# SchlomoFeng/GDN

Hardware: AMD Instinct MI355X
Metric: sliding-windows/sec forward+anomaly-score, SWaT-shape (127 sensors, W=15) (higher is better)
Workload: dtype f32; 1 GPU; BASELINE configs[2]: SWaT-shape eval forward + anomaly score; sensors=127, window=15, topk=30, dim=64, out_layer_num=1, batch=512, batches_per_launch=64, windows_per_launch=32768, storage=fp32, multi_gpu_measured=False, hip_graph=True, forward_streams=3, parallelism=single GPU

## Files before the change

gdn_amd/_lib.py:

```python
from __future__ import annotations

import ctypes
import functools
import os

_HERE = os.path.dirname(os.path.abspath(__file__))
LIB_PATH = os.environ.get("GDN_HIP_LIB", os.path.join(_HERE, "libgdn_hip.so"))
ABI_VERSION = 23

_c_int, _c_float, _p = ctypes.c_int, ctypes.c_float, ctypes.c_void_p

SIGNATURES = {
    "gdn_abi_version": [],
    "gdn_nbr_pitch": [_c_int],
    "gdn_topk_graph": [_p, _c_int, _c_int, _c_int, _p, _p, _p, _p, _p],
    "gdn_graph_from_topk": [_p, _c_int, _c_int, _p, _p, _p],
    "gdn_node_terms": [_p, _p, _p, _p, _p, _p, _c_int, _c_int, _c_int, _p, _p],
    "gdn_bn_fold": [_p, _p, _p, _p, _c_float, _c_int, _p, _p],
    "gdn_project_fwd": [_p, _p, _p, _c_int, _c_int, _c_int, _c_int, _p, _p, _p, _p],
    "gdn_project_fwd_series": [_p, _c_int, _c_int, _p, _p, _c_int, _c_int, _c_int, _c_int, _p, _p, _p, _p],
    "gdn_tile_fits": [_c_int] * 4,
    "gdn_kernel_family": [_c_int] * 6,
    "gdn_tile_forward_form": [_c_int] * 5,
    "gdn_terms_pitch": [_c_int],
    "gdn_attn_aggregate_fwd": [_p, _p, _p, _p, _p, _p, _c_int, _c_int, _c_int, _c_int, _p, _p, _p],
    "gdn_head_fwd": [_p, _p, _p, _p, _p, _p, _c_int, _c_int, _c_int, _p, _p, _p],
    "gdn_head_train_fwd": [_p] * 10 + [_c_float] + [_c_int] * 3 + [_c_float] * 4 + [_p] * 9,
    "gdn_head_train_workspace_bytes": [_c_int, _c_int],
    "gdn_head_train_stats_bytes": [_c_int],
    "gdn_exact_sum_workspace_bytes": [],
    "gdn_exact_sum": [_p, _c_int, _p, _p, _p],
    "gdn_head_train_bwd": [_p] * 10 + [_c_float, _p] + [_c_int] * 3 + [_c_float] * 2 + [_p] * 10,
    "gdn_head_train_fwd_rng": [_p] * 9 + [_c_float] + [_c_int] * 3 + [_c_float] * 4 + [_p] * 8 + [_c_int, _p],
    "gdn_head_train_bwd_rng": [_p] * 9 + [_c_float, _p] + [_c_int] * 3 + [_c_float] * 2 + [_p] * 9 + [_c_int, _p],
    "gdn_head_train_fwd_act": [_p] * 8 + [_c_float, _p, _c_float] + [_c_int] * 3 + [_c_float] * 4 + [_p] * 8 + [_c_int, _p],
    "gdn_head_train_bwd_act": [_p] * 9 + [_c_float, _p, _c_float, _p] + [_c_int] * 3 + [_c_float] * 2 + [_p] * 7 + [_c_int, _p],
    "gdn_mlp_train_saved_bytes": [_c_int] * 4,
    "gdn_mlp_train_workspace_bytes": [_c_int] * 4,
    "gdn_mlp_train_fwd": [_p] * 8 + [_c_int] * 4 + [_p] * 4,
    "gdn_mlp_train_bwd": [_p] * 4 + [_c_int] * 4 + [_p] * 7,
    "gdn_mlp_eval_workspace_bytes": [_c_int] * 4,
    "gdn_mlp_eval_fwd": [_p] * 6 + [_c_int] * 4 + [_p] * 3,
    "gdn_topk_graph_terms": [_p, _c_int, _c_int, _c_int] + [_p] * 8 + [_c_int, _p, _p],
    "gdn_forward_fused_plan_keys": [_p] * 4 + [_c_int] * 7 + [_p, _p],
    "gdn_forward_fused_series_plan_keys": [_p, _c_int, _c_int] + [_p] * 3 + [_c_int] * 6 + [_p, _p],
    "gdn_attn_aggregate_bwd_uses_reverse": [_c_int] * 3,
    "gdn_head_mse_workspace_bytes": [],
    "gdn_head_train_fwd_rng_mse": [_p] * 9 + [_c_float] + [_c_int] * 3 + [_c_float] * 4 + [_p] * 12 + [_c_int, _p],
    "gdn_project_bwd_partials": [_p] * 4 + [_c_int] * 4 + [_p, _p, _p],
    "gdn_train_finish": [_p, _p] + [_c_int] * 4 + [_p] * 8 + [_c_int, _c_int] + [_p] * 4,
    "gdn_adam_step": [_p] * 5 + [_c_int] + [ctypes.c_double] * 6 + [_c_int, _c_int, _p],
    "gdn_terms_bwd_acc": [_p] * 8 + [_c_int] * 3 + [_p] * 6 + [_c_int, _p],
    "gdn_mse_workspace_bytes": [],
    "gdn_mse_loss_grad": [_p, _p, ctypes.c_longlong, _p, _p, _p, _p],
    "gdn_forward_fused": [_p] * 11 + [_c_int] * 5 + [_p, _p],
    "gdn_forward_fused_series": [_p, _c_int, _c_int] + [_p] * 10 + [_c_int] * 5 + [_p, _p],
    "gdn_mlp_plan_bytes": [_c_int] * 3,
    "gdn_mlp_plan_layer": [_p] * 6 + [_c_float] + [_c_int] * 4 + [_p, _p],
    "gdn_mlp_plan_out": [_p, _p] + [_c_int] * 3 + [_p, _p],
    "gdn_mlp_fwd": [_p, _p] + [_c_int] * 4 + [_p, _p],
    "gdn_head_mlp_fwd": [_p] * 5 + [_c_int] * 5 + [_p, _p],
    "gdn_fused_plan_bytes": [_c_int] * 5,
    "gdn_fused_plan_build": [_p] * 10 + [_c_int] * 5 + [_p, _p],
    "gdn_forward_fused_plan": [_p, _p] + [_c_int] * 6 + [_p, _p, _p],
    "gdn_forward_fused_series_plan": [_p, _c_int, _c_int, _p] + [_c_int] * 5 + [_p, _p, _p],
    "gdn_fused_plan_limit_offset": [_c_int] * 5,
    "gdn_graph_bank_order": [_p, _c_int, _c_int, _p, _p],
    "gdn_forward_fused_gated": [_p] * 12 + [_c_int] * 5 + [_p, _p],
    "gdn_forward_fused_series_gated": [_p, _p, _c_int, _c_int] + [_p] * 10 + [_c_int] * 5 + [_p, _p],
    "gdn_project_fwd_wide": [_p, _p, _p, _c_int, _c_int, _c_int, _c_int, _p, _p, _p, _p],
    "gdn_attn_aggregate_fwd_wide": [_p, _p, _p, _p, _p, _p, _c_int, _c_int, _c_int, _c_int, _p, _p, _p],
    "gdn_attn_aggregate_bwd_wide": [_p] * 8 + [_c_int] * 4 + [_p] * 6,
    "gdn_project_fwd_bf16": [_p, _p, _p, _c_int, _c_int, _c_int, _c_int, _p, _p, _p, _p],
    "gdn_attn_aggregate_fwd_bf16": [_p, _p, _p, _p, _p, _p, _c_int, _c_int, _c_int, _c_int, _p, _p, _p],
    "gdn_head_fwd_bf16": [_p, _p, _p, _p, _p, _p, _c_int, _c_int, _c_int, _p, _p, _p],
    "gdn_forward_fused_bf16": [_p] * 11 + [_c_int] * 5 + [_p, _p],
    "gdn_attn_aggregate_bwd": [_p] * 8 + [_c_int] * 4 + [_p] * 6,
    "gdn_attn_aggregate_bwd_workspace_bytes": [_c_int] * 4,
    "gdn_train_supported": [_c_int] * 4,
    "gdn_rev_pitch": [_c_int],
    "gdn_graph_reverse": [_p, _p, _c_int, _c_int, _p, _p, _p],
    "gdn_project_bwd_workspace_bytes": [_c_int, _c_int, _c_int],
    "gdn_project_bwd": [_p] * 4 + [_c_int] * 4 + [_p] * 5,
    "gdn_terms_bwd": [_p] * 8 + [_c_int] * 3 + [_p] * 7,
    "gdn_score_workspace_bytes": [_c_int, _c_int],
    "gdn_score_select_workspace_bytes": [_c_int, _c_int, _c_int],
    "gdn_score_keys": [_p, _p, _c_int, _c_int, _c_int, _p, _p],
    "gdn_score_select": [_p, _c_int, _c_int, _c_int, ctypes.c_longlong, _p, _p, _p],
    "gdn_score_select_paths": [_p, _c_int, _c_int, _c_int, ctypes.c_longlong, _p, _p, _p, _p],
    "gdn_score_quantiles": [_p, _p, _c_int, _c_int, _p, _p, _p],
    "gdn_score_smooth_max": [_p, _p, _p, _c_int, _c_int, _c_int, _p, _p, _p, _p, _p],
    "gdn_score_smooth_topm": [_p, _p, _p, _c_int, _c_int, _c_int, _p, _p, _c_int, _p, _p, _p],
    "gdn_series_fill_workspace_bytes": [_c_int, _c_int],
    "gdn_series_fill": [_p] + [_c_int] * 3 + [_p] * 7,
    "gdn_score_keys_keep": [_p, _p, _p, _c_int, _c_int, _c_int, _p, _p],
    "gdn_score_smooth_max_gaps": [_p, _p, _p, _c_int, _c_int, _c_int, _p, _p, _p, _p, _p, _p, _p],
    "gdn_score_smooth_topm_gaps": [_p, _p, _p, _c_int, _c_int, _c_int, _p, _p, _c_int, _p, _p, _p, _p, _p],
    "gdn_attention_workspace_bytes": [_c_int] * 4,
    "gdn_attention_mean": [_p, ctypes.c_longlong, ctypes.c_longlong] + [_p] * 4 + [_c_int] * 4 + [_p, _p, _p],
    "gdn_attention_at": [_p, ctypes.c_longlong, _p, _p, _c_int, _p, _p, _p] + [_c_int] * 3 + [_p, _p],
    "gdn_windows_gather": [_p, _c_int, ctypes.c_longlong, _p, ctypes.c_longlong, _p, ctypes.c_longlong, _c_int, _c_int,
                           _p, _p, _p],
    "gdn_epoch_advance": [_p, _p, _p, ctypes.c_longlong, _p],
    "gdn_mse_batch_means": [_p, _p, ctypes.c_longlong, _c_int, ctypes.c_longlong, _p, _p, _p, _p],
    "gdn_windows_gather_gaps": [_p, _c_int, ctypes.c_longlong, _p, ctypes.c_longlong, _p, ctypes.c_longlong, _c_int,
                                _c_int, _p, _p, _p, _p, _p, _p],
    "gdn_mse_batch_means_masked": [_p, _p, _p, ctypes.c_longlong, _c_int, ctypes.c_longlong, _p, _p, _p, _p, _p],
    "gdn_mse_loss_grad_masked": [_p, _p, _p, _p, _c_int, _c_int, _p, _p, _p, _p, _p],
    "gdn_stream_state_bytes": [_c_int, _c_int],
    "gdn_stream_init": [_p, _p, ctypes.c_longlong, _c_int, _c_int, _p],
    "gdn_stream_windows": [_p, _p, _c_int, _c_int, _c_int, _c_int, _p, _p],
    "gdn_stream_score": [_p] * 5 + [_c_int] * 4 + [_p] * 4,
    "gdn_stream_advance": [_p] * 6 + [_c_int] * 5 + [_p, _p, ctypes.c_longlong, _p],
    "gdn_stream_fill": [_p, _p] + [_c_int] * 4 + [_p] * 4,
    "gdn_stream_score_gaps": [_p] * 6 + [_c_int] * 4 + [_p] * 4,
    "gdn_stream_advance_gaps": [_p] * 8 + [_c_int] * 5 + [_p, _p, ctypes.c_longlong, _p, _p],
    "gdn_stream_calib_bytes": [_c_int, _c_int],
    "gdn_stream_calib_write": [_p] * 4 + [_c_int] * 5 + [_p] * 3,
    "gdn_stream_calib_write_gaps": [_p] * 5 + [_c_int] * 5 + [_p] * 3,
    "gdn_score_keys_valid": [_p, _p, _p, _c_int, _c_int, _c_int, _p, _p],
    "gdn_score_key_counts": [_p, _c_int, _c_int, _c_int, _p, _p],
    "gdn_score_select_counts": [_p, _c_int, _c_int, _c_int, _p, _c_int, _p, _p, _p, _p],
    "gdn_stream_calib_write_sensor": [_p] * 5 + [_c_int] * 5 + [_p] * 3,
    "gdn_prep_stats_workspace_bytes": [ctypes.c_longlong, _c_int],
    "gdn_prep_stats": [_p, ctypes.c_longlong, _c_int, _c_int, _p, _p, _p],
    "gdn_prep_series": [_p, ctypes.c_longlong, _c_int, _c_int, _p, _p, _c_int, _p, _p, _p, _p],
    "gdn_prep_ticks": [_p, _c_int, _c_int, _p, _c_int, _p, _c_int, _c_int, _p, _p, _c_int, _p],
    "gdn_episodes_workspace_bytes": [ctypes.c_longlong, ctypes.c_longlong],
    "gdn_episodes_scan": [_p, _p, ctypes.c_longlong, _c_int, ctypes.c_double, ctypes.c_double, _c_int, _c_int,
                          ctypes.c_longlong, ctypes.c_longlong] + [_p] * 10,
    "gdn_episodes_scan_grid": [_p, _p, ctypes.c_longlong, _c_int, ctypes.c_double, ctypes.c_double, _c_int, _c_int,
                               ctypes.c_longlong, ctypes.c_longlong] + [_p] * 9 + [_c_int, _p],
    "gdn_stream_events_bytes": [_c_int, ctypes.c_longlong],
    "gdn_stream_events": [_p] * 5 + [_c_int] * 5 + [ctypes.c_longlong, _p, _p],
    "gdn_alarm_sweep": [_p, _p, ctypes.c_longlong, _p, _p, _p, _p, ctypes.c_longlong, _p, _p],
    "gdn_fleet_state_bytes": [_c_int] * 3,
    "gdn_fleet_init": [_p, _p, ctypes.c_longlong, _c_int, _c_int, _c_int, _p],
    "gdn_fleet_windows": [_p] * 3 + [_c_int] * 4 + [_p, _p],
    "gdn_fleet_score": [_p] * 6 + [_c_int] * 5 + [_p] * 4,
    "gdn_fleet_advance": [_p] * 7 + [_c_int] * 5 + [_p, _p, ctypes.c_longlong, _p],
    "gdn_fleet_fill": [_p] * 3 + [_c_int] * 4 + [_p] * 4,
    "gdn_fleet_score_gaps": [_p] * 7 + [_c_int] * 5 + [_p] * 4,
    "gdn_fleet_advance_gaps": [_p] * 9 + [_c_int] * 5 + [_p, _p, ctypes.c_longlong, _p, _p],
    "gdn_fleet_events_bytes": [_c_int, _c_int, ctypes.c_longlong],
    "gdn_fleet_events": [_p] * 6 + [_c_int] * 7 + [ctypes.c_longlong, _p, _p],
    "gdn_fleet_calib_bytes": [_c_int] * 3,
    "gdn_fleet_calib_write": [_p] * 5 + [_c_int] * 6 + [_p] * 3,
    "gdn_fleet_calib_write_gaps": [_p] * 6 + [_c_int] * 6 + [_p] * 3,
    "gdn_fleet_calib_write_sensor": [_p] * 6 + [_c_int] * 6 + [_p] * 3,
    "gdn_fleet_ring_counts": [_p, _p, _c_int, _c_int, _c_int, _p, _p, _p],
    "gdn_fleet_ring_threshold_bytes": [_c_int, _c_int],
    "gdn_fleet_ring_threshold": [_p] * 5 + [_c_int] * 5 + [ctypes.c_double, _c_int] + [_p] * 8,
    "gdn_fleet_prep_bytes": [_c_int] * 3,
    "gdn_fleet_prep_ticks": [_p, _c_int, _c_int, _p, _p] + [_c_int] * 4 + [_p] * 4,
}

FAMILY_NONE, FAMILY_DENSE, FAMILY_TILE, FAMILY_LARGE, FAMILY_LONG, FAMILY_ANY = range(6)
STAGE_PROJECT, STAGE_AGGREGATE, STAGE_ATTN_BWD, STAGE_PROJECT_BWD, STAGE_TERMS, STAGE_HEAD, STAGE_FUSED = range(7)
ROUTE_WIDE, ROUTE_BF16, ROUTE_SERIES = 1, 2, 4


@functools.lru_cache(maxsize=None)
def family(stage: int, n: int, w: int, d: int, k: int, flags: int = 0) -> int:
    return load().gdn_kernel_family(stage, n, w, d, k, flags) & 0xff


ERRORS = {-1: "GDN_ERR_ARG (null pointer or non-positive dimension)",
          -2: "GDN_ERR_LAUNCH (HIP launch failed)",
          -3: "GDN_ERR_UNSUPPORTED (shape outside the supported set, see include/gdn_hip.h)"}

_lib = None


class GdnHipError(RuntimeError):
    pass


def load() -> ctypes.CDLL:
    global _lib
    if _lib is not None:
        return _lib
    if not os.path.exists(LIB_PATH):
        raise GdnHipError(
            f"{LIB_PATH} not found: the HIP extension is not built and gdn_amd has no CPU "
            "fallback. Run `python -c \"import __graft_entry__ as g; g.build()\"` (needs hipcc).")
    lib = ctypes.CDLL(LIB_PATH)
    for name, argtypes in SIGNATURES.items():
        fn = getattr(lib, name)
        fn.argtypes = argtypes
        fn.restype = ctypes.c_longlong if name.endswith(("_bytes", "_offset")) else _c_int
    if lib.gdn_abi_version() != ABI_VERSION:
        raise GdnHipError(f"ABI mismatch: library {lib.gdn_abi_version()} != binding {ABI_VERSION}")
    _lib = lib
    return lib


def call(name: str, *args) -> None:
    rc = getattr(load(), name)(*args)
    if rc != 0:
        raise GdnHipError(f"{name} failed: {ERRORS.get(rc, rc)}")
```

gdn_amd/csrc/gdn_forward_dense.hip:

```cpp
#include "gdn_common.hpp"

#include <stdlib.h>

int gdn_dense_fused_op_d128(int op, const void* args, int bf16, unsigned* plan_out, long long* bytes,
                            hipStream_t st);

namespace {

typedef _Float16 h8 __attribute__((ext_vector_type(8)));
typedef _Float16 h2 __attribute__((ext_vector_type(2)));
typedef __bf16 b8 __attribute__((ext_vector_type(8)));
typedef __bf16 b2 __attribute__((ext_vector_type(2)));
typedef float f32x16 __attribute__((ext_vector_type(16)));
typedef unsigned int u32x4 __attribute__((ext_vector_type(4)));
typedef float f32x2 __attribute__((ext_vector_type(2)));

#ifndef GDN_TRIM_SPLIT
#define GDN_TRIM_SPLIT 1
#endif
#ifndef GDN_TRIM_RELU
#define GDN_TRIM_RELU 1
#endif
#ifndef GDN_TRIM_PACK
#define GDN_TRIM_PACK 1
#endif

template <bool PACK>
struct Pk2 {
  static __device__ __forceinline__ f32x2 mul(f32x2 a, f32x2 b) {
    if constexpr (PACK) return a * b;
    return f32x2{a[0] * b[0], a[1] * b[1]};
  }
  static __device__ __forceinline__ f32x2 mul(f32x2 a, float b) { return mul(a, f32x2{b, b}); }
  static __device__ __forceinline__ f32x2 add(f32x2 a, f32x2 b) {
    if constexpr (PACK) return a + b;
    return f32x2{a[0] + b[0], a[1] + b[1]};
  }
  static __device__ __forceinline__ f32x2 add(f32x2 a, float b) { return add(a, f32x2{b, b}); }
  static __device__ __forceinline__ f32x2 sub(f32x2 a, float b) {
    if constexpr (PACK) return a - f32x2{b, b};
    return f32x2{a[0] - b, a[1] - b};
  }
  static __device__ __forceinline__ f32x2 fma(f32x2 a, f32x2 b, f32x2 c) {
    if constexpr (PACK) return __builtin_elementwise_fma(a, b, c);
    return f32x2{__builtin_fmaf(a[0], b[0], c[0]), __builtin_fmaf(a[1], b[1], c[1])};
  }
};

__device__ __forceinline__ float relu_acc(float v) {
#if GDN_TRIM_RELU
  return __builtin_elementwise_maximum(v, 0.f);
#else
  return fmaxf(v, 0.f);
// ... 54 lines not shown
    hi = __builtin_bit_cast(unsigned, p);
    lo = __builtin_bit_cast(unsigned, l);
  }
  static __device__ __forceinline__ f32x16 mfma(u32x4 a, u32x4 b, f32x16 c) {
    return __builtin_amdgcn_mfma_f32_32x32x16_f16(__builtin_bit_cast(h8, a), __builtin_bit_cast(h8, b), c, 0, 0, 0);
  }
};

template <>
struct Fmt<FMT_BF16> {
  static __device__ __forceinline__ unsigned pk(float a, float b) {
    asm("" : "+v"(a));
    asm("" : "+v"(b));
    const b2 p = {(__bf16)a, (__bf16)b};
    return __builtin_bit_cast(unsigned, p);
  }
  static __device__ __forceinline__ float res0(unsigned p, float x) { return x - __uint_as_float(p << 16); }
  static __device__ __forceinline__ float res1(unsigned p, float x) { return x - __uint_as_float(p & 0xffff0000u); }
  static __device__ __forceinline__ void split2(float& a, float& b, unsigned& hi, unsigned& lo) {
    hi = pk(a, b);
    lo = pk(res0(hi, a), res1(hi, b));
  }
  static __device__ __forceinline__ f32x16 mfma(u32x4 a, u32x4 b, f32x16 c) {
    return __builtin_amdgcn_mfma_f32_32x32x16_bf16(__builtin_bit_cast(b8, a), __builtin_bit_cast(b8, b), c, 0, 0, 0);
  }
};

template <int FMT, int NTERM, bool TRIM = true>
__device__ __forceinline__ void split8(const float (&v)[8], u32x4 (&out)[NTERM]) {
  float r[8];
#pragma unroll
  for (int j = 0; j < 8; ++j) r[j] = v[j];
  if constexpr (NTERM == 2 && TRIM) {
#pragma unroll
    for (int j = 0; j < 4; ++j) {
      unsigned hi, lo;
      Fmt<FMT>::split2(r[2 * j], r[2 * j + 1], hi, lo);
      out[0][j] = hi;
      out[NTERM - 1][j] = lo;
    }
    return;
  }
#pragma unroll
  for (int t = 0; t < NTERM; ++t)
#pragma unroll
    for (int j = 0; j < 4; ++j) {
      const unsigned p = Fmt<FMT>::pk(r[2 * j], r[2 * j + 1]);
      out[t][j] = p;
      if (t + 1 < NTERM) {
        r[2 * j] = Fmt<FMT>::res0(p, r[2 * j]);
        r[2 * j + 1] = Fmt<FMT>::res1(p, r[2 * j + 1]);
      }
    }
}

__host__ __device__ __forceinline__ int pos_of_source(int src) {
  return (src & ~12) | ((src & 4) << 1) | ((src & 8) >> 1);
}

enum { DMODE_FUSED = 0 };

template <int NT, int DC, int WK, int SL, int FMT>
struct DCfg {
  static constexpr int KS = 2 * NT;
  static constexpr int ROWS = 32 * NT;
  static constexpr int THREADS = 64 * NT;
  static constexpr int AROW = KS * 32 + 16;
  static constexpr int AWAVE = 32 * AROW;
  static constexpr bool XAGG = FMT == FMT_F16;
  static constexpr int MCB = XAGG ? 1 : DC;
  static constexpr int NPX = FMT == FMT_F16 ? 2 : 1;
  static constexpr int NTL = FMT == FMT_F16 ? 2 : 3;
  static constexpr int NTXIN = FMT == FMT_F16 ? 2 : 1;
  static constexpr int XP = 16 * WK + 4;
  static constexpr int XU = 8 * WK;
  static constexpr bool XHALF = XAGG && WK == 1;
  static constexpr int XFL = XHALF ? 16 : 32;
  static constexpr int XFRAG = 2 * XFL * 16;
  static constexpr int OFF_A = 0;
  static constexpr int OFF_XF = NT * AWAVE;
  static constexpr int OFF_XS = OFF_XF + KS * MCB * NPX * XFRAG;
  static constexpr int OFF_SI = OFF_XS + (XAGG ? 0 : ROWS * XP * 4);
  static constexpr int OFF_SJ = OFF_SI + ROWS * 4;
  static constexpr int OFF_EC = OFF_SJ + ROWS * 4;
  static constexpr int OFF_CS = OFF_EC + 4 * 32 * DC * 4;
  static constexpr int CS_WORDS = XAGG ? 0 : 3 * ROWS;
  static constexpr bool XKFAM = XHALF && DC == 2 && SL <= 16;
  static constexpr int XKEEP_TABLE = SL <= 8 || NT == 4 ? KS : 2;
  static constexpr int XKEEP = !XKFAM ? 0 : GDN_XKEEP < 0 ? XKEEP_TABLE : GDN_XKEEP < KS ? GDN_XKEEP : KS;
  static constexpr bool BLDS = XKFAM && (GDN_BL_LDS < 0 ? SL > 8 && NT == 4 : GDN_BL_LDS != 0);
  static constexpr int OFF_BL = OFF_CS + CS_WORDS * 4;
  static constexpr int LDS = OFF_BL + (BLDS ? DC * WK * NTL * 1024 : 0);
  static constexpr int CW = 16 * WK, RS = THREADS / CW;
  static __host__ __device__ constexpr int xrow0(int xsl) { return XAGG ? 16 * (xsl >> 1) + 4 * (xsl & 1) : xsl; }
  static __host__ __device__ constexpr int xro(int u) {
    return XAGG ? 16 * NT * (u >> 3) + 8 * ((u & 7) >> 2) + (u & 3) : u * RS;
  }
  static constexpr int LDS_UNIT = 1280;
  static constexpr int LDS_ALLOC = (LDS + LDS_UNIT - 1) / LDS_UNIT * LDS_UNIT;
  static constexpr bool PACK = GDN_TRIM_PACK != 0 && SL <= 16 && FMT == FMT_F16;
  static constexpr int WGS = !(DC == 2 && NT >= 3 && SL <= 16 && WK == 1) ? 1
                             : XAGG && 3 * LDS_ALLOC <= 160 * 1024 ? 3 : 2;
};

struct DArgs {
  const void* x;
  int series_len;
  int series_first;
  int batch, n, w, pitch, d;
  const float* lin_w;
// ... 227 lines not shown
    for (int r = 0; r < 16; ++r) {
      const int c = cb * 32 + (r & 3) + 8 * (r >> 2) + 4 * h;
      k.e2[cb][r] = ld_or(a.emb, tgt * d + c, tgt < n) * a.bn2[c] *
                    (FMT == FMT_F16 ? 1.f / (GDN_F16_Z_SCALE * GDN_F16_X_SCALE) : 1.f);
    }
  k.out_b = a.out_b[0];
}

template <int NT, int DC, int FMT>
__device__ __forceinline__ void compute_tables(const DArgs& a, float* dst) {
  constexpr int ROWS = 32 * NT, THREADS = 64 * NT, d = 32 * DC;
  const int tid = threadIdx.x, n = a.n;
  for (int c = tid; c < d; c += THREADS) {
    dst[c] = a.bn2[d + c];
    dst[d + c] = a.out_w[c];
    dst[2 * d + c] = a.bn1[c];
    dst[3 * d + c] = fmaf(a.gnn_bias[c], a.bn1[c], a.bn1[d + c]) *
                     (FMT == FMT_F16 ? GDN_F16_Z_SCALE * GDN_F16_X_SCALE : 1.f);
  }
  if constexpr (FMT == FMT_F16) return;
  float* ct = dst + 4 * d;
  for (int t = tid; t < 3 * ROWS; t += THREADS) {
    const int which = t / ROWS, row = t - which * ROWS;
    float v = ld_or(a.node_terms, 2 * GDN_A_PITCH + which * n + row, which < 2 && row < n) * GDN_LOG2E;
    if (which == 1 && row == n) v = -INFINITY;
    ct[t] = v;
  }
}

template <int NT, int DC, int FMT>
__device__ __forceinline__ float compute_xlimit(const DArgs& a) {
  if constexpr (FMT != FMT_F16) return INFINITY;
  __shared__ unsigned m_lin, m_c;
  const int tid = threadIdx.x, d = 32 * DC;
  if (tid == 0) { m_lin = 0u; m_c = 0u; }
  __syncthreads();
  for (int c = tid; c < d; c += 64 * NT) {
    const float sc = a.bn1[c] * GDN_F16_X_SCALE;
    float lmax = 0.f;
    for (int q = 0; q < a.w; ++q) {
      const float v = fabsf(a.lin_w[c * a.w + q] * sc);
      lmax = v > lmax || v != v ? v : lmax;
    }
    const float cin = fabsf(fmaf(a.gnn_bias[c], a.bn1[c], a.bn1[d + c]));
    atomicMax(&m_lin, __float_as_uint(lmax));
    atomicMax(&m_c, __float_as_uint(cin));
  }
  __syncthreads();
  const float lmax = __uint_as_float(m_lin), cmax = __uint_as_float(m_c);
  if (!(lmax < 60000.f) || !(cmax < 3.0e38f)) return 0.f;
  return 60000.f / GDN_F16_XT_SCALE;
}

template <int NT, int DC, int WK, int SL, int FMT>
__global__ __launch_bounds__(64 * NT) void gdn_dense_plan_kernel(const DArgs a, unsigned* plan) {
  using K = LaneConsts<NT, DC, WK, SL, FMT>;
  constexpr int T = 64 * NT;
  __shared__ int s_sj[T][SL], s_sc[T][SL];
  __shared__ unsigned char s_perm[T][SL];
  K k;
  compute_lane_consts(a, k);
  const int tid = threadIdx.x;
#pragma unroll
  for (int q = 0; q < SL; ++q) {
    s_sj[tid][q] = k.sjoff[q];
    s_sc[tid][q] = k.scoff[q];
  }
  __syncthreads();
  if ((tid & 31) == 0) {
    unsigned used[32];
    for (int l = 0; l < 32; ++l) used[l] = 0;
    for (int step = 0; step < SL; ++step) {
      unsigned char cw[32], cr[32];
      for (int i = 0; i < 32; ++i) cw[i] = cr[i] = 0;
      for (int l = 0; l < 32; ++l) {
        int best = -1, best_cost = 1 << 30;
        for (int q = 0; q < SL; ++q) {
          if (used[l] >> q & 1u) continue;
          const int bw = (s_sc[tid + l][q] >> 2) & 31, br = (s_sj[tid + l][q] >> 2) & 31;
          const int cost = 2 * (cw[bw] >= 1 ? 1 + 4 * (cw[bw] - 1) : 0) + (cr[br] >= 1 ? 1 + 4 * (cr[br] - 1) : 0);
          if (cost < best_cost) { best_cost = cost; best = q; }
        }
        used[l] |= 1u << best;
        s_perm[tid + l][step] = (unsigned char)best;
        ++cw[(s_sc[tid + l][best] >> 2) & 31];
        ++cr[(s_sj[tid + l][best] >> 2) & 31];
      }
    }
  }
  __syncthreads();
#pragma unroll
  for (int q = 0; q < SL; ++q) {
    k.sjoff[q] = s_sj[tid][s_perm[tid][q]];
    k.scoff[q] = s_sc[tid][s_perm[tid][q]];
  }
  compute_tables<NT, DC, FMT>(a, reinterpret_cast<float*>(plan));
  unsigned* lanes = plan + K::TABLE_WORDS;
  k.each_word([&](int i, unsigned& wd) { lanes[i * T + threadIdx.x] = wd; });
  const float xlim = compute_xlimit<NT, DC, FMT>(a);
  if (threadIdx.x == 0) plan[K::LIMIT_WORD] = __float_as_uint(xlim);
}

#ifndef GDN_DENSE_EXTRA_DC
template <int NT, int SL>
__global__ __launch_bounds__(64 * NT) void gdn_bank_order_kernel(const uint16_t* __restrict__ nbr, int n, int pitch,
                                                                 uint16_t* __restrict__ out) {
  constexpr int T = 64 * NT;
  __shared__ unsigned short s_j[T][SL];
  __shared__ unsigned char s_perm[T][SL];
  const int tid = threadIdx.x, lane = tid & 63, wv = tid >> 6;
  const int ti = 32 * wv + (lane >> 1), half = lane & 1;
  const uint16_t* row = nbr + (size_t)min(ti, n - 1) * pitch + half * SL;
#pragma unroll
  for (int q = 0; q < SL; ++q) s_j[tid][q] = ti < n ? row[q] : (unsigned short)n;
  __syncthreads();
  if ((tid & 31) == 0) {
    unsigned used[32];
    for (int l = 0; l < 32; ++l) used[l] = 0;
    for (int step = 0; step < SL; ++step) {
      unsigned char cw[32], cr[32];
      for (int i = 0; i < 32; ++i) cw[i] = cr[i] = 0;
      for (int l = 0; l < 32; ++l) {
        const int rowdw = (((tid + l) & 63) >> 1) * (16 * NT + 4);
        int best = -1, best_cost = 1 << 30;
        for (int q = 0; q < SL; ++q) {
          if (used[l] >> q & 1u) continue;
          const int j = s_j[tid + l][q];
          const int bw = (rowdw + (pos_of_source(j) >> 1)) & 31, br = j & 31;
          const int cost = 2 * (cw[bw] >= 1 ? 1 + 4 * (cw[bw] - 1) : 0) + (cr[br] >= 1 ? 1 + 4 * (cr[br] - 1) : 0);
          if (cost < best_cost) { best_cost = cost; best = q; }
        }
        used[l] |= 1u << best;
        s_perm[tid + l][step] = (unsigned char)best;
        const int jb = s_j[tid + l][best];
        ++cw[(rowdw + (pos_of_source(jb) >> 1)) & 31];
        ++cr[jb & 31];
      }
    }
  }
  __syncthreads();
  if (ti < n) {
    uint16_t* dst = out + (size_t)ti * pitch + half * SL;
#pragma unroll
    for (int q = 0; q < SL; ++q) dst[q] = s_j[tid][s_perm[tid][q]];
  }
}
#endif

#ifdef GDN_DENSE_EXTRA_DC
#define GDN_FUSED_ATTR __attribute__((amdgpu_waves_per_eu(1, 1)))
#else
#define GDN_FUSED_ATTR
#endif
#ifndef GDN_K8_PRIO_T
#define GDN_K8_PRIO_T 2
#define GDN_K8_PRIO_S 0
#define GDN_K8_PRIO_M 3
#define GDN_K8_PRIO_Z 1
#endif
#ifndef GDN_PRIO_P
#define GDN_PRIO_P 2
#define GDN_PRIO_S 0
#define GDN_PRIO_M 3
#define GDN_PRIO_E 1
#endif
#ifndef GDN_PRIO_P1
#define GDN_PRIO_P1 3
#endif
template <int NT, int DC, int WK, int SL, int FMT>
__global__ __launch_bounds__(64 * NT, (DCfg<NT, DC, WK, SL, FMT>::WGS)) GDN_FUSED_ATTR void gdn_dense_fused_kernel(const DArgs a) {
  using C = DCfg<NT, DC, WK, SL, FMT>;
  using F = Fmt<FMT>;
  using P = Pk2<C::PACK>;
  extern __shared__ uint4 smem_u4[];
  char* smem = reinterpret_cast<char*>(smem_u4);
  const int tid = threadIdx.x, lane = tid & 63, wv = tid >> 6;
  const int l32 = lane & 31, h = lane >> 5;
  const int n = a.n, w = a.w, d = 32 * DC;
  constexpr bool FOLD = FMT == FMT_F16;
  GDN_STAMP(0)

  for (int t = lane; t < C::AWAVE / 16; t += 64)
    reinterpret_cast<uint4*>(smem + C::OFF_A + wv * C::AWAVE)[t] = make_uint4(0, 0, 0, 0);
  {
  }
  LaneConsts<NT, DC, WK, SL, FMT> k;
  float xlim = INFINITY;
  if (a.plan) {
    const unsigned* lanes = a.plan + LaneConsts<NT, DC, WK, SL, FMT>::TABLE_WORDS;
    k.each_word([&](int i, unsigned& wd) { wd = lanes[i * C::THREADS + tid]; });
    unsigned* tab = reinterpret_cast<unsigned*>(smem + C::OFF_EC);
    for (int t = tid; t < LaneConsts<NT, DC, WK, SL, FMT>::TABLE_WORDS; t += C::THREADS) tab[t] = a.plan[t];
    if constexpr (FMT == FMT_F16)
      if (a.range_flag) xlim = __uint_as_float(a.plan[LaneConsts<NT, DC, WK, SL, FMT>::LIMIT_WORD]);
  } else {
    compute_lane_consts(a, k);
    compute_tables<NT, DC, FMT>(a, reinterpret_cast<float*>(smem + C::OFF_EC));
  }
// ... 1247 lines not shown
}

static int fused_dispatch(int op, const DArgs& a, int bf16, unsigned* plan_out, long long* bytes, hipStream_t st) {
  if (a.d == 128) return gdn_dense_fused_op_d128(op, &a, bf16, plan_out, bytes, st);
  return bf16 ? select_nt<FMT_BF16, 2>(op, a, plan_out, bytes, st) : select_nt<FMT_F16, 2>(op, a, plan_out, bytes, st);
}

int gdn_dense_forward_fused(const void* x, int x_is_bf16, int series_len, int series_first, const float* lin_w,
                            const float* node_terms, const uint16_t* nbr, const float* gnn_bias,
                            const float* emb, const float* bn1, const float* bn2, const float* out_w,
                            const float* out_b, int batch, int n, int w, int d, int k, float* out,
                            hipStream_t stream) {
  if (!gdn_dense_fused_supported(n, w, d, k)) return GDN_ERR_UNSUPPORTED;
  DArgs a = {};
  a.x = x; a.series_len = series_len; a.series_first = series_first;
  a.batch = batch; a.n = n; a.w = w; a.pitch = gdn_nbr_pitch(k); a.d = d;
  a.lin_w = lin_w; a.node_terms = node_terms; a.nbr = nbr; a.gnn_bias = gnn_bias; a.emb = emb;
  a.bn1 = bn1; a.bn2 = bn2; a.out_w = out_w; a.out_b = out_b; a.out = out;
  return fused_dispatch(DOP_LAUNCH, a, x_is_bf16, nullptr, nullptr, stream);
}

#ifdef GDN_STAMPS
extern "C" int gdn_debug_read_stamps(unsigned long long* host_out) {
  return hipMemcpyFromSymbol(host_out, HIP_SYMBOL(g_dense_stamps), sizeof(g_dense_stamps)) == hipSuccess ? 0 : -2;
}
#endif

template <int NT>
static int bank_order_select_sl(const uint16_t* nbr, int n, int pitch, uint16_t* out, hipStream_t st) {
  switch (pitch) {
    case 16: hipLaunchKernelGGL((gdn_bank_order_kernel<NT, 8>), dim3(1), dim3(64 * NT), 0, st, nbr, n, pitch, out); break;
    case 32: hipLaunchKernelGGL((gdn_bank_order_kernel<NT, 16>), dim3(1), dim3(64 * NT), 0, st, nbr, n, pitch, out); break;
    case 48: hipLaunchKernelGGL((gdn_bank_order_kernel<NT, 24>), dim3(1), dim3(64 * NT), 0, st, nbr, n, pitch, out); break;
    case 64: hipLaunchKernelGGL((gdn_bank_order_kernel<NT, 32>), dim3(1), dim3(64 * NT), 0, st, nbr, n, pitch, out); break;
    default: return GDN_ERR_UNSUPPORTED;
  }
  return gdn_launch_status();
}

extern "C" int gdn_graph_bank_order(const uint16_t* nbr, int n, int k, uint16_t* nbr_ordered, void* stream) {
  if (!nbr || !nbr_ordered || n <= 0 || k <= 0) return GDN_ERR_ARG;
  if (!gdn_dense_supported(n, 1, 64, k)) return GDN_ERR_UNSUPPORTED;
  const int pitch = gdn_nbr_pitch(k);
  hipStream_t st = (hipStream_t)stream;
  switch ((n + 1 + 31) / 32) {
    case 1: return bank_order_select_sl<1>(nbr, n, pitch, nbr_ordered, st);
    case 2: return bank_order_select_sl<2>(nbr, n, pitch, nbr_ordered, st);
    case 3: return bank_order_select_sl<3>(nbr, n, pitch, nbr_ordered, st);
    case 4: return bank_order_select_sl<4>(nbr, n, pitch, nbr_ordered, st);
  }
  return GDN_ERR_UNSUPPORTED;
}

extern "C" long long gdn_fused_plan_bytes(int n, int w, int d, int k, int bf16_storage) {
  if (!gdn_dense_fused_supported(n, w, d, k)) return 0;
  DArgs a = {};
  a.n = n; a.w = w; a.d = d; a.pitch = gdn_nbr_pitch(k);
  long long bytes = 0;
  const int rc = fused_dispatch(DOP_PLAN_BYTES, a, bf16_storage, nullptr, &bytes, nullptr);
  return rc == GDN_OK ? bytes : 0;
}

extern "C" int gdn_fused_plan_build(const float* lin_w, const float* node_terms, const uint16_t* nbr,
                                    const int32_t* deg, const float* gnn_bias, const float* emb,
                                    const float* bn1_affine, const float* bn2_affine, const float* out_w,
                                    const float* out_b, int n, int w, int d, int k, int bf16_storage,
                                    void* plan, void* stream) {
  if (!lin_w || !node_terms || !nbr || !deg || !gnn_bias || !emb || !bn1_affine || !bn2_affine || !out_w ||
      !out_b || !plan)
    return GDN_ERR_ARG;
  if (!gdn_dense_fused_supported(n, w, d, k)) return GDN_ERR_UNSUPPORTED;
  DArgs a = {};
  a.n = n; a.w = w; a.d = d; a.pitch = gdn_nbr_pitch(k);
  a.lin_w = lin_w; a.node_terms = node_terms; a.nbr = nbr; a.gnn_bias = gnn_bias; a.emb = emb;
  a.bn1 = bn1_affine; a.bn2 = bn2_affine; a.out_w = out_w; a.out_b = out_b;
  unsigned* p = reinterpret_cast<unsigned*>(plan);
  return fused_dispatch(DOP_PLAN_BUILD, a, bf16_storage, p, nullptr, (hipStream_t)stream);
}

static int fused_with_plan(const void* x, int series_len, int first, const void* plan, int batch, int n, int w,
                           int d, int k, int bf16_storage, float* out, void* stream, const float* key_gt = nullptr,
                           double* keys = nullptr, int key_pitch = 0, int* range_guard = nullptr) {
  if (!x || !plan || !out) return GDN_ERR_ARG;
  if (batch <= 0 || n <= 0) return GDN_ERR_ARG;
  if (keys && (!key_gt || key_pitch < batch)) return GDN_ERR_ARG;
  if (!gdn_dense_fused_supported(n, w, d, k)) return GDN_ERR_UNSUPPORTED;
  DArgs a = {};
  a.x = x; a.series_len = series_len; a.series_first = first;
  a.batch = batch; a.n = n; a.w = w; a.pitch = gdn_nbr_pitch(k); a.d = d;
  a.out = out; a.plan = reinterpret_cast<const unsigned*>(plan);
  a.key_gt = key_gt; a.keys = keys; a.key_pitch = key_pitch;
  a.range_flag = bf16_storage ? nullptr : range_guard;
  return fused_dispatch(DOP_LAUNCH, a, bf16_storage, nullptr, nullptr, (hipStream_t)stream);
}

extern "C" int gdn_forward_fused_plan(const void* x, const void* plan, int batch, int n, int w, int d, int k,
                                      int bf16_storage, float* out, int* range_guard, void* stream) {
  return fused_with_plan(x, 0, 0, plan, batch, n, w, d, k, bf16_storage, out, stream, nullptr, nullptr, 0, range_guard);
}

extern "C" int gdn_forward_fused_series_plan(const float* series, int series_len, int first, const void* plan,
                                             int batch, int n, int w, int d, int k, float* out, int* range_guard,
                                             void* stream) {
  if (series_len <= 0 || first < 0 || (long long)first + batch - 1 + w > series_len) return GDN_ERR_ARG;
  return fused_with_plan(series, series_len, first, plan, batch, n, w, d, k, 0, out, stream, nullptr, nullptr, 0,
                         range_guard);
// ... 23 lines not shown
```

include/gdn_hip.h:

```cpp
#ifndef GDN_HIP_H
#define GDN_HIP_H

#include <stdint.h>

#ifdef __cplusplus
extern "C" {
#endif

#define GDN_OK 0
#define GDN_ERR_ARG (-1)
#define GDN_ERR_LAUNCH (-2)
#define GDN_ERR_UNSUPPORTED (-3)

#define GDN_ABI_VERSION 23
int gdn_abi_version(void);

int gdn_nbr_pitch(int k);

int gdn_topk_graph(const float* emb, int n, int d, int k,
                   int64_t* topk_idx, uint16_t* nbr, int32_t* deg, float* cos_out, void* stream);

int gdn_graph_from_topk(const int64_t* topk_idx, int n, int k,
                        uint16_t* nbr, int32_t* deg, void* stream);

// ... 126 lines not shown
                           const float* mask, const uint8_t* keep, float keep_scale,
                           const long long* rng_seed_step, float p_drop,
                           const double* stats, int batch, int n, int d, float eps1, float eps2,
                           double* workspace, float* d_z, float* d_emb, float* d_bn1_w, float* d_bn1_b,
                           float* d_bn2_w, float* d_bn2_b, int buffers_zeroed, void* stream);
long long gdn_mlp_train_saved_bytes(int rows, int d_in, int hidden, int layers);
long long gdn_mlp_train_workspace_bytes(int rows, int d_in, int hidden, int layers);
int gdn_mlp_train_fwd(const float* act, const float* const* params, float* const* running,
                      long long* const* batches, const float* eps, const float* momentum,
                      const float* out_w, const float* out_b, int rows, int d_in, int hidden,
                      int layers, void* saved, void* workspace, float* out, void* stream);
int gdn_mlp_train_bwd(const float* d_out, const float* act, const float* const* params,
                      const float* out_w, int rows, int d_in, int hidden, int layers,
                      const void* saved, void* workspace, float* const* grads, float* d_out_w,
                      float* d_out_b, float* d_act, void* stream);

long long gdn_mlp_eval_workspace_bytes(int rows, int d_in, int hidden, int layers);
int gdn_mlp_eval_fwd(const float* act, const float* const* params, const float* const* running,
                     const float* eps, const float* out_w, const float* out_b,
                     int rows, int d_in, int hidden, int layers, void* workspace, float* out, void* stream);

int gdn_project_bwd_partials(const float* x, const float* d_xlin, const float* d_si, const float* d_sj,
                             int batch, int n, int w, int d, float* workspace, int* rows_out,
                             void* stream);
int gdn_train_finish(double* head_workspace, double* stats, int head_zeroed, int batch, int n, int d,
                     float* d_emb, float* d_bn1_w, float* d_bn1_b, float* d_bn2_w, float* d_bn2_b,
                     float* d_lin_w, float* d_lin_b, const float* proj_workspace, int proj_rows, int w,
                     float* d_proj_w, float* d_a, float* d_c, void* stream);

int gdn_adam_step(float* params, float* grads, float* exp_avg, float* exp_avg_sq,
                  long long* step, int count, double lr, double beta1, double beta2, double eps,
                  double weight_decay, double grad_scale, int zero_from, int zero_count, void* stream);

long long gdn_mse_workspace_bytes(void);
int gdn_mse_loss_grad(const float* out, const float* y, long long count, double* workspace,
                      float* loss, float* d_out, void* stream);

int gdn_mse_loss_grad_masked(const float* out, const float* y, const uint8_t* valid, const int* row_valid, int batch,
                             int n, double* workspace, float* loss, float* d_out, int64_t* m_out, void* stream);

int gdn_forward_fused(const float* x, const float* lin_w, const float* node_terms,
                      const uint16_t* nbr, const int32_t* deg, const float* gnn_bias,
                      const float* emb, const float* bn1_affine, const float* bn2_affine,
                      const float* out_w, const float* out_b,
                      int batch, int n, int w, int d, int k, float* out, void* stream);

int gdn_forward_fused_series(const float* series, int series_len, int first, const float* lin_w,
                             const float* node_terms, const uint16_t* nbr, const int32_t* deg,
                             const float* gnn_bias, const float* emb, const float* bn1_affine,
                             const float* bn2_affine, const float* out_w, const float* out_b,
                             int batch, int n, int w, int d, int k, float* out, void* stream);

int gdn_graph_bank_order(const uint16_t* nbr, int n, int k, uint16_t* nbr_ordered, void* stream);

long long gdn_fused_plan_bytes(int n, int w, int d, int k, int bf16_storage);
int gdn_fused_plan_build(const float* lin_w, const float* node_terms, const uint16_t* nbr,
                         const int32_t* deg, const float* gnn_bias, const float* emb,
                         const float* bn1_affine, const float* bn2_affine, const float* out_w,
                         const float* out_b, int n, int w, int d, int k, int bf16_storage,
                         void* plan, void* stream);
int gdn_forward_fused_plan(const void* x, const void* plan, int batch, int n, int w, int d, int k,
                           int bf16_storage, float* out, int* range_guard, void* stream);
int gdn_forward_fused_series_plan(const float* series, int series_len, int first, const void* plan,
                                  int batch, int n, int w, int d, int k, float* out, int* range_guard,
                                  void* stream);

long long gdn_fused_plan_limit_offset(int n, int w, int d, int k, int bf16_storage);
int gdn_forward_fused_gated(int* guard, const float* x, const float* lin_w, const float* node_terms,
                            const uint16_t* nbr, const int32_t* deg, const float* gnn_bias,
                            const float* emb, const float* bn1_affine, const float* bn2_affine,
                            const float* out_w, const float* out_b,
                            int batch, int n, int w, int d, int k, float* out, void* stream);
int gdn_forward_fused_series_gated(int* guard, const float* series, int series_len, int first,
                                   const float* lin_w, const float* node_terms, const uint16_t* nbr,
                                   const int32_t* deg, const float* gnn_bias, const float* emb,
                                   const float* bn1_affine, const float* bn2_affine, const float* out_w,
                                   const float* out_b, int batch, int n, int w, int d, int k, float* out,
                                   void* stream);
int gdn_project_fwd_wide(const float* x, const float* lin_w, const float* node_terms,
                         int batch, int n, int w, int d,
                         float* xlin, float* s_i, float* s_j, void* stream);
int gdn_attn_aggregate_fwd_wide(const float* xlin, const float* s_i, const float* s_j,
                                const uint16_t* nbr, const int32_t* deg, const float* bias,
                                int batch, int n, int d, int k,
                                float* z, float* alpha, void* stream);
int gdn_attn_aggregate_bwd_wide(const float* d_z, const float* xlin, const float* alpha,
                                const float* s_i, const float* s_j,
                                const uint16_t* nbr, const uint32_t* rent, const int32_t* rlen,
                                int batch, int n, int d, int k,
                                float* d_xlin, float* d_si, float* d_sj, float* d_bias,
                                float* workspace, void* stream);

int gdn_forward_fused_plan_keys(const void* x, const void* plan, const float* gt, double* keys,
                                int key_pitch, int batch, int n, int w, int d, int k, int bf16_storage,
                                float* out, void* stream);
int gdn_forward_fused_series_plan_keys(const float* series, int series_len, int first, const void* plan,
                                       const float* gt, double* keys, int key_pitch, int batch, int n,
                                       int w, int d, int k, float* out, void* stream);

int gdn_project_fwd_bf16(const uint16_t* x, const float* lin_w, const float* node_terms,
                         int batch, int n, int w, int d,
                         uint16_t* xlin, float* s_i, float* s_j, void* stream);
int gdn_attn_aggregate_fwd_bf16(const uint16_t* xlin, const float* s_i, const float* s_j,
                                const uint16_t* nbr, const int32_t* deg, const float* bias,
                                int batch, int n, int d, int k,
                                uint16_t* z, float* alpha, void* stream);
// ... 205 lines not shown
```

Measured before the change: 154.8 million windows/s.

## Refine LDS bank-conflict slot ordering with pairwise swap local search

Replaces the greedy per-lane slot ordering used in plan building and neighbour bank ordering with a shared routine. The routine does the same greedy pass and then runs rounds of cost-reducing pairwise slot swaps, using incremental read/write bank-conflict histograms. The aim is fewer LDS bank conflicts in the fused forward kernel's gather and scatter steps. It also adds a host entry point that computes the same ordering and reports its conflict cost. The extra search runs only in the one-time plan or ordering kernels, so the per-window cost changes only through the better slot order.

```diff
diff --git a/gdn_amd/_lib.py b/gdn_amd/_lib.py
--- a/gdn_amd/_lib.py
+++ b/gdn_amd/_lib.py
@@ -66,6 +66,7 @@
     "gdn_forward_fused_series_plan": [_p, _c_int, _c_int, _p] + [_c_int] * 5 + [_p, _p, _p],
     "gdn_fused_plan_limit_offset": [_c_int] * 5,
     "gdn_graph_bank_order": [_p, _c_int, _c_int, _p, _p],
+    "gdn_bank_order_host": [_p, _c_int, _c_int, _p, _c_int, _p],
     "gdn_forward_fused_gated": [_p] * 12 + [_c_int] * 5 + [_p, _p],
     "gdn_forward_fused_series_gated": [_p, _p, _c_int, _c_int] + [_p] * 10 + [_c_int] * 5 + [_p, _p],
     "gdn_project_fwd_wide": [_p, _p, _p, _c_int, _c_int, _c_int, _c_int, _p, _p, _p, _p],
@@ -165,6 +166,8 @@
     return load().gdn_kernel_family(stage, n, w, d, k, flags) & 0xff
 
 
+HOST_ONLY_ADDITIONS = {"gdn_bank_order_host"}
+
 ERRORS = {-1: "GDN_ERR_ARG (null pointer or non-positive dimension)",
           -2: "GDN_ERR_LAUNCH (HIP launch failed)",
           -3: "GDN_ERR_UNSUPPORTED (shape outside the supported set, see include/gdn_hip.h)"}
@@ -186,6 +189,8 @@
             "fallback. Run `python -c \"import __graft_entry__ as g; g.build()\"` (needs hipcc).")
     lib = ctypes.CDLL(LIB_PATH)
     for name, argtypes in SIGNATURES.items():
+        if name in HOST_ONLY_ADDITIONS and "GDN_HIP_LIB" in os.environ and not hasattr(lib, name):
+            continue
         fn = getattr(lib, name)
         fn.argtypes = argtypes
         fn.restype = ctypes.c_longlong if name.endswith(("_bytes", "_offset")) else _c_int
diff --git a/gdn_amd/csrc/gdn_bank_order.hpp b/gdn_amd/csrc/gdn_bank_order.hpp
--- /dev/null
+++ b/gdn_amd/csrc/gdn_bank_order.hpp
@@ -0,0 +1,194 @@
+#pragma once
+#include <stdint.h>
+
+#ifndef __HIPCC__
+#define __host__
+#define __device__
+#endif
+
+#define BANK_ORDER_MAX_ROUNDS 48
+
+__host__ __device__ inline int pos_of_source(int src) {
+  return (src & ~12) | ((src & 4) << 1) | ((src & 8) >> 1);
+}
+
+__host__ __device__ inline int bank_order_write_bank(int lane, int j, int nt) {
+  return (((lane & 63) >> 1) * (16 * nt + 4) + (pos_of_source(j) >> 1)) & 31;
+}
+
+template <int SL>
+struct BankOrderGroup {
+  uint8_t j[32][SL];
+  uint8_t wb[32][SL];
+  uint8_t perm[32][SL];
+  uint8_t rc[SL][128];
+  uint8_t rd[SL][32];
+  uint8_t wc[SL][32];
+  uint8_t rh[SL][8];
+  uint8_t wh[SL][20];
+  uint8_t rmax[SL], wmax[SL];
+  uint32_t used[32];
+  uint8_t gr[32];
+  int32_t prop[32];
+};
+
+__host__ __device__ inline int bank_step_cost(const uint8_t (&jj)[32], const uint8_t (&wb)[32]) {
+  int rmax = 1, wmax = 1;
+  for (int b = 0; b < 32; ++b) {
+    unsigned seen = 0;
+    int writers = 0;
+    for (int l = 0; l < 32; ++l) {
+      if ((jj[l] & 31) == b) seen |= 1u << (jj[l] >> 5);
+      writers += wb[l] == b;
+    }
+    const int r = (int)(seen & 1) + (int)(seen >> 1 & 1) + (int)(seen >> 2 & 1) + (int)(seen >> 3 & 1);
+    rmax = r > rmax ? r : rmax;
+    wmax = (writers + 1) / 2 > wmax ? (writers + 1) / 2 : wmax;
+  }
+  return (rmax - 1) + 2 * (wmax - 1);
+}
+
+template <int SL>
+__host__ __device__ inline int group_cost(const BankOrderGroup<SL>& g) {
+  int cost = 0;
+  for (int s = 0; s < SL; ++s) {
+    uint8_t jj[32], wb[32];
+    for (int l = 0; l < 32; ++l) {
+      jj[l] = g.j[l][g.perm[l][s]];
+      wb[l] = g.wb[l][g.perm[l][s]];
+    }
+    cost += bank_step_cost(jj, wb);
+  }
+  return cost;
+}
+
+namespace bank_order_detail {
+
+template <int SL>
+__host__ __device__ inline void move_entry(BankOrderGroup<SL>& g, int s, int j, int wb, int dir) {
+  const int b = j & 31;
+  const int c = g.rc[s][j];
+  g.rc[s][j] = (uint8_t)(c + dir);
+  if (dir > 0 ? c == 0 : c == 1) {
+    const int d = g.rd[s][b];
+    g.rd[s][b] = (uint8_t)(d + dir);
+    --g.rh[s][d];
+    ++g.rh[s][d + dir];
+    if (d + dir > g.rmax[s]) g.rmax[s] = (uint8_t)(d + dir);
+    else if (g.rh[s][g.rmax[s]] == 0) --g.rmax[s];
+  }
+  const int w = g.wc[s][wb];
+  g.wc[s][wb] = (uint8_t)(w + dir);
+  const int lo = (w + 1) >> 1, ln = (w + dir + 1) >> 1;
+  if (lo != ln) {
+    --g.wh[s][lo];
+    ++g.wh[s][ln];
+    if (ln > g.wmax[s]) g.wmax[s] = (uint8_t)ln;
+    else if (g.wh[s][g.wmax[s]] == 0) --g.wmax[s];
+  }
+}
+
+__host__ __device__ inline int max_after(const uint8_t* hist, int m, int ao, int an, int bo, int bn) {
+  if (an > m || bn > m) return m + 1;
+  const int at_m = hist[m] - (ao == m && an != m) - (bo == m && bn != m) + (an == m && ao != m) + (bn == m && bo != m);
+  return at_m > 0 ? m : m - 1;
+}
+
+template <int SL>
+__host__ __device__ inline int replace_delta(const BankOrderGroup<SL>& g, int s, int j0, int w0, int j1, int w1) {
+  int delta = 0;
+  if (j0 != j1) {
+    const int b0 = j0 & 31, b1 = j1 & 31;
+    const int down = g.rc[s][j0] == 1, up = g.rc[s][j1] == 0;
+    int ao = g.rd[s][b0], an = ao - down, bo = g.rd[s][b1], bn = bo + up;
+    if (b0 == b1) {
+      an = ao - down + up;
+      bo = bn = 0;
+    }
+    const int m = g.rmax[s];
+    delta += ((max_after(g.rh[s], m, ao, an, bo, bn) - m) << 16) + an * an - ao * ao + bn * bn - bo * bo;
+  }
+  if (w0 != w1) {
+    const int ao = (g.wc[s][w0] + 1) >> 1, an = g.wc[s][w0] >> 1;
+    const int bo = (g.wc[s][w1] + 1) >> 1, bn = (g.wc[s][w1] + 2) >> 1;
+    const int m = g.wmax[s];
+    delta += 2 * (((max_after(g.wh[s], m, ao, an, bo, bn) - m) << 16) + an * an - ao * ao + bn * bn - bo * bo);
+  }
+  return delta;
+}
+
+}
+
+template <int SL, class Sync>
+__host__ __device__ inline void bank_order_group(BankOrderGroup<SL>& g, int lane0, int lanes, int method,
+                                                 Sync&& any_sync) {
+  using namespace bank_order_detail;
+  static_assert(SL <= 32, "a lane's slots are a 32-bit set");
+  any_sync(false);
+  if (lane0 == 0) {
+    for (int s = 0; s < SL; ++s) {
+      for (int a = 0; a < 128; ++a) g.rc[s][a] = 0;
+      for (int b = 0; b < 32; ++b) g.rd[s][b] = g.wc[s][b] = 0;
+      for (int v = 0; v < 8; ++v) g.rh[s][v] = 0;
+      for (int v = 0; v < 20; ++v) g.wh[s][v] = 0;
+      g.rh[s][0] = g.wh[s][0] = 32;
+      g.rmax[s] = g.wmax[s] = 0;
+    }
+    for (int l = 0; l < 32; ++l) g.used[l] = 0;
+    for (int s = 0; s < SL; ++s) {
+      for (int b = 0; b < 32; ++b) g.gr[b] = 0;
+      for (int l = 0; l < 32; ++l) {
+        int best = -1, best_cost = 1 << 30;
+        const uint32_t used = g.used[l];
+        for (int q = 0; q < SL; ++q) {
+          if (used >> q & 1u) continue;
+          const int cw = g.wc[s][g.wb[l][q]], c = g.gr[g.j[l][q] & 31];
+          const int cost = 2 * (cw >= 1 ? 1 + 4 * (cw - 1) : 0) + (c >= 1 ? 1 + 4 * (c - 1) : 0);
+          if (cost < best_cost) { best_cost = cost; best = q; }
+        }
+        g.used[l] = used | 1u << best;
+        g.perm[l][s] = (uint8_t)best;
+        ++g.gr[g.j[l][best] & 31];
+        move_entry(g, s, g.j[l][best], g.wb[l][best], +1);
+      }
+    }
+  }
+  any_sync(false);
+  if (method == 0) return;
+  for (int round = 0; round < BANK_ORDER_MAX_ROUNDS; ++round) {
+    bool proposed = false;
+    for (int l = lane0; l < 32; l += lanes) {
+      int best = 0, best_pair = -1;
+      for (int s1 = 0; s1 < SL; ++s1) {
+        const int q1 = g.perm[l][s1], j1 = g.j[l][q1], w1 = g.wb[l][q1];
+        for (int s2 = s1 + 1; s2 < SL; ++s2) {
+          const int q2 = g.perm[l][s2], j2 = g.j[l][q2], w2 = g.wb[l][q2];
+          if (g.rd[s1][j1 & 31] < 2 && g.wc[s1][w1] < 3 && g.rd[s2][j2 & 31] < 2 && g.wc[s2][w2] < 3) continue;
+          const int delta = replace_delta(g, s1, j1, w1, j2, w2) + replace_delta(g, s2, j2, w2, j1, w1);
+          if (delta < best) { best = delta; best_pair = s1 << 8 | s2; }
+        }
+      }
+      g.prop[l] = best_pair;
+      proposed |= best_pair >= 0;
+    }
+    if (!any_sync(proposed)) break;
+    if (lane0 == 0) {
+      uint32_t touched = 0;
+      for (int l = 0; l < 32; ++l) {
+        const int pair = g.prop[l];
+        if (pair < 0) continue;
+        const int s1 = pair >> 8, s2 = pair & 255;
+        if (touched >> s1 & 1u || touched >> s2 & 1u) continue;
+        touched |= 1u << s1 | 1u << s2;
+        const int q1 = g.perm[l][s1], q2 = g.perm[l][s2];
+        move_entry(g, s1, g.j[l][q1], g.wb[l][q1], -1);
+        move_entry(g, s1, g.j[l][q2], g.wb[l][q2], +1);
+        move_entry(g, s2, g.j[l][q2], g.wb[l][q2], -1);
+        move_entry(g, s2, g.j[l][q1], g.wb[l][q1], +1);
+        g.perm[l][s1] = (uint8_t)q2;
+        g.perm[l][s2] = (uint8_t)q1;
+      }
+    }
+    any_sync(false);
+  }
+}
diff --git a/gdn_amd/csrc/gdn_forward_dense.hip b/gdn_amd/csrc/gdn_forward_dense.hip
--- a/gdn_amd/csrc/gdn_forward_dense.hip
+++ b/gdn_amd/csrc/gdn_forward_dense.hip
@@ -1,4 +1,5 @@
 #include "gdn_common.hpp"
+#include "gdn_bank_order.hpp"
 
 #include <stdlib.h>
 
@@ -159,10 +160,6 @@
         r[2 * j + 1] = Fmt<FMT>::res1(p, r[2 * j + 1]);
       }
     }
-}
-
-__host__ __device__ __forceinline__ int pos_of_source(int src) {
-  return (src & ~12) | ((src & 4) << 1) | ((src & 8) >> 1);
 }
 
 enum { DMODE_FUSED = 0 };
@@ -496,47 +493,38 @@
   return 60000.f / GDN_F16_XT_SCALE;
 }
 
+template <int NT, int SL>
+__device__ __forceinline__ void order_slots(int (&j)[SL]) {
+  __shared__ BankOrderGroup<SL> s_groups[2 * NT];
+  const int tid = threadIdx.x, l = tid & 31;
+  BankOrderGroup<SL>& g = s_groups[tid >> 5];
+#pragma unroll
+  for (int q = 0; q < SL; ++q) {
+    g.j[l][q] = (uint8_t)j[q];
+    g.wb[l][q] = (uint8_t)bank_order_write_bank(tid, j[q], NT);
+  }
+  bank_order_group<SL>(g, l, 32, 1, [](bool changed) { return __syncthreads_or(changed) != 0; });
+#pragma unroll
+  for (int q = 0; q < SL; ++q) j[q] = g.j[l][g.perm[l][q]];
+}
+
 template <int NT, int DC, int WK, int SL, int FMT>
 __global__ __launch_bounds__(64 * NT) void gdn_dense_plan_kernel(const DArgs a, unsigned* plan) {
+  using C = DCfg<NT, DC, WK, SL, FMT>;
   using K = LaneConsts<NT, DC, WK, SL, FMT>;
   constexpr int T = 64 * NT;
-  __shared__ int s_sj[T][SL], s_sc[T][SL];
-  __shared__ unsigned char s_perm[T][SL];
+  static_assert(C::OFF_SJ % 128 == 0 && C::OFF_A % 128 == 0 && C::AWAVE % 128 == 0 && C::AROW == 4 * (16 * NT + 4), "");
   K k;
   compute_lane_consts(a, k);
-  const int tid = threadIdx.x;
+  const int tid = threadIdx.x, lane = tid & 63, wv = tid >> 6;
+  int j[SL];
+#pragma unroll
+  for (int q = 0; q < SL; ++q) j[q] = (k.sjoff[q] - C::OFF_SJ) >> 2;
+  order_slots<NT, SL>(j);
 #pragma unroll
   for (int q = 0; q < SL; ++q) {
-    s_sj[tid][q] = k.sjoff[q];
-    s_sc[tid][q] = k.scoff[q];
-  }
-  __syncthreads();
-  if ((tid & 31) == 0) {
-    unsigned used[32];
-    for (int l = 0; l < 32; ++l) used[l] = 0;
-    for (int step = 0; step < SL; ++step) {
-      unsigned char cw[32], cr[32];
-      for (int i = 0; i < 32; ++i) cw[i] = cr[i] = 0;
-      for (int l = 0; l < 32; ++l) {
-        int best = -1, best_cost = 1 << 30;
-        for (int q = 0; q < SL; ++q) {
-          if (used[l] >> q & 1u) continue;
-          const int bw = (s_sc[tid + l][q] >> 2) & 31, br = (s_sj[tid + l][q] >> 2) & 31;
-          const int cost = 2 * (cw[bw] >= 1 ? 1 + 4 * (cw[bw] - 1) : 0) + (cr[br] >= 1 ? 1 + 4 * (cr[br] - 1) : 0);
-          if (cost < best_cost) { best_cost = cost; best = q; }
-        }
-        used[l] |= 1u << best;
-        s_perm[tid + l][step] = (unsigned char)best;
-        ++cw[(s_sc[tid + l][best] >> 2) & 31];
-        ++cr[(s_sj[tid + l][best] >> 2) & 31];
-      }
-    }
-  }
-  __syncthreads();
-#pragma unroll
-  for (int q = 0; q < SL; ++q) {
-    k.sjoff[q] = s_sj[tid][s_perm[tid][q]];
-    k.scoff[q] = s_sc[tid][s_perm[tid][q]];
+    k.sjoff[q] = C::OFF_SJ + j[q] * 4;
+    k.scoff[q] = C::OFF_A + wv * C::AWAVE + (lane >> 1) * C::AROW + pos_of_source(j[q]) * 2;
   }
   compute_tables<NT, DC, FMT>(a, reinterpret_cast<float*>(plan));
   unsigned* lanes = plan + K::TABLE_WORDS;
@@ -549,45 +537,45 @@
 template <int NT, int SL>
 __global__ __launch_bounds__(64 * NT) void gdn_bank_order_kernel(const uint16_t* __restrict__ nbr, int n, int pitch,
                                                                  uint16_t* __restrict__ out) {
-  constexpr int T = 64 * NT;
-  __shared__ unsigned short s_j[T][SL];
-  __shared__ unsigned char s_perm[T][SL];
   const int tid = threadIdx.x, lane = tid & 63, wv = tid >> 6;
   const int ti = 32 * wv + (lane >> 1), half = lane & 1;
   const uint16_t* row = nbr + (size_t)min(ti, n - 1) * pitch + half * SL;
-#pragma unroll
-  for (int q = 0; q < SL; ++q) s_j[tid][q] = ti < n ? row[q] : (unsigned short)n;
-  __syncthreads();
-  if ((tid & 31) == 0) {
-    unsigned used[32];
-    for (int l = 0; l < 32; ++l) used[l] = 0;
-    for (int step = 0; step < SL; ++step) {
-      unsigned char cw[32], cr[32];
-      for (int i = 0; i < 32; ++i) cw[i] = cr[i] = 0;
-      for (int l = 0; l < 32; ++l) {
-        const int rowdw = (((tid + l) & 63) >> 1) * (16 * NT + 4);
-        int best = -1, best_cost = 1 << 30;
-        for (int q = 0; q < SL; ++q) {
-          if (used[l] >> q & 1u) continue;
-          const int j = s_j[tid + l][q];
-          const int bw = (rowdw + (pos_of_source(j) >> 1)) & 31, br = j & 31;
-          const int cost = 2 * (cw[bw] >= 1 ? 1 + 4 * (cw[bw] - 1) : 0) + (cr[br] >= 1 ? 1 + 4 * (cr[br] - 1) : 0);
-          if (cost < best_cost) { best_cost = cost; best = q; }
-        }
-        used[l] |= 1u << best;
-        s_perm[tid + l][step] = (unsigned char)best;
-        const int jb = s_j[tid + l][best];
-        ++cw[(rowdw + (pos_of_source(jb) >> 1)) & 31];
-        ++cr[jb & 31];
-      }
-    }
-  }
-  __syncthreads();
+  int j[SL];
+#pragma unroll
+  for (int q = 0; q < SL; ++q) j[q] = ti < n ? (int)row[q] : n;
+  order_slots<NT, SL>(j);
   if (ti < n) {
     uint16_t* dst = out + (size_t)ti * pitch + half * SL;
 #pragma unroll
-    for (int q = 0; q < SL; ++q) dst[q] = s_j[tid][s_perm[tid][q]];
-  }
+    for (int q = 0; q < SL; ++q) dst[q] = (uint16_t)j[q];
+  }
+}
+
+template <int SL>
+static long long bank_order_host(const uint16_t* nbr, int n, int pitch, uint16_t* out, int method) {
+  const int nt = (n + 1 + 31) / 32;
+  long long cost = 0;
+  BankOrderGroup<SL>* g = new BankOrderGroup<SL>;
+  for (int grp = 0; grp < 2 * nt; ++grp) {
+    for (int l = 0; l < 32; ++l) {
+      const int tid = 32 * grp + l, lane = tid & 63, ti = 32 * (tid >> 6) + (lane >> 1);
+      const uint16_t* row = nbr + (size_t)(ti < n ? ti : n - 1) * pitch + (lane & 1) * SL;
+      for (int q = 0; q < SL; ++q) {
+        const int j = ti < n ? (int)row[q] : n;
+        g->j[l][q] = (uint8_t)j;
+        g->wb[l][q] = (uint8_t)bank_order_write_bank(tid, j, nt);
+      }
+    }
+    bank_order_group<SL>(*g, 0, 1, method, [](bool changed) { return changed; });
+    cost += group_cost(*g);
+    for (int l = 0; l < 32; ++l) {
+      const int tid = 32 * grp + l, lane = tid & 63, ti = 32 * (tid >> 6) + (lane >> 1);
+      if (ti >= n) continue;
+      for (int q = 0; q < SL; ++q) out[(size_t)ti * pitch + (lane & 1) * SL + q] = g->j[l][g->perm[l][q]];
+    }
+  }
+  delete g;
+  return cost;
 }
 #endif
 
@@ -1941,6 +1929,22 @@
   return GDN_ERR_UNSUPPORTED;
 }
 
+extern "C" int gdn_bank_order_host(const uint16_t* nbr, int n, int k, uint16_t* out, int method, long long* cost) {
+  if (!nbr || !out || n <= 0 || k <= 0 || (method != 0 && method != 1)) return GDN_ERR_ARG;
+  if (!gdn_dense_supported(n, 1, 64, k)) return GDN_ERR_UNSUPPORTED;
+  const int pitch = gdn_nbr_pitch(k);
+  long long c = 0;
+  switch (pitch) {
+    case 16: c = bank_order_host<8>(nbr, n, pitch, out, method); break;
+    case 32: c = bank_order_host<16>(nbr, n, pitch, out, method); break;
+    case 48: c = bank_order_host<24>(nbr, n, pitch, out, method); break;
+    case 64: c = bank_order_host<32>(nbr, n, pitch, out, method); break;
+    default: return GDN_ERR_UNSUPPORTED;
+  }
+  if (cost) *cost = c;
+  return GDN_OK;
+}
+
 extern "C" long long gdn_fused_plan_bytes(int n, int w, int d, int k, int bf16_storage) {
   if (!gdn_dense_fused_supported(n, w, d, k)) return 0;
   DArgs a = {};
diff --git a/include/gdn_hip.h b/include/gdn_hip.h
--- a/include/gdn_hip.h
+++ b/include/gdn_hip.h
@@ -202,6 +202,8 @@
                              int batch, int n, int w, int d, int k, float* out, void* stream);
 
 int gdn_graph_bank_order(const uint16_t* nbr, int n, int k, uint16_t* nbr_ordered, void* stream);
+
+int gdn_bank_order_host(const uint16_t* nbr, int n, int k, uint16_t* out, int method, long long* cost);
 
 long long gdn_fused_plan_bytes(int n, int w, int d, int k, int bf16_storage);
 int gdn_fused_plan_build(const float* lin_w, const float* node_terms, const uint16_t* nbr,
```

After: 156.0 million windows/s (median of 6 runs). Within noise of the previous version (+0.8%).
